# i2Nav-WHU/IC-GVINS

Measured on AMD Instinct MI355X. Metric: frames/s at 1280x720, 300 feats, 10-KF window; residual/Jacobian eval/s, higher is better.
Workload: dtype u8/int64 front-end (f32/f64 solves), f64 factors

## Files before the change

### ic-gvins_amd/csrc/ctx.hip

```cpp
#include <algorithm>
#include <cstdarg>

#include <sys/prctl.h>
#include <time.h>

#include "icg_internal.h"

int icg_fail(icg_ctx *ctx, int code, const char *fmt, ...) {
    char buf[512];
    va_list ap;
    va_start(ap, fmt);
    vsnprintf(buf, sizeof buf, fmt, ap);
    va_end(ap);
    if (ctx) ctx->err = buf;
    return code;
}

int icg_hip_check(icg_ctx *ctx, hipError_t e, const char *what) {
    if (e == hipSuccess) return 0;
    return icg_fail(ctx, ICG_ERR_HIP, "HIP error %d (%s) at %s", (int) e, hipGetErrorString(e), what);
}

static thread_local std::string g_create_error;

extern "C" const char *icg_version(void) { return "icgvins-hip 0.1 (gfx950)"; }

extern "C" const char *icg_last_error(const icg_ctx *ctx) { return ctx ? ctx->err.c_str() : g_create_error.c_str(); }

int icg_stream_wait_poll(icg_ctx *ctx) {
    static thread_local bool slack_set = false;
    if (!slack_set) {
        (void) prctl(PR_SET_TIMERSLACK, 1000UL, 0, 0, 0);
        slack_set = true;
    }
    struct timespec ts = {0, ctx->poll_sleep_ns};
    for (int it = 0;; it++) {
        hipError_t e = hipStreamQuery(ctx->stream);
        if (e == hipSuccess) return ICG_OK;
        if (e != hipErrorNotReady) return icg_hip_check(ctx, e, "hipStreamQuery");
        if (it >= 4) nanosleep(&ts, nullptr);
    }
}

extern "C" int icg_ctx_set_wait_mode(icg_ctx *ctx, int mode, int sleep_us) {
    if (!ctx || (mode != ICG_WAIT_SPIN && mode != ICG_WAIT_POLL) || (mode == ICG_WAIT_POLL && sleep_us <= 0)) return ICG_ERR_INVALID;
    if (ctx->wait_mode_env) return ICG_OK;
    ctx->poll_sleep_ns = mode == ICG_WAIT_POLL ? 1000L * sleep_us : 0;
    return ICG_OK;
}

icg_pyr_desc icg_make_pyr_desc(const icg_ctx *ctx) {
    icg_pyr_desc d{};
    d.base       = ctx->d_frames;
    d.slot_bytes = ctx->slot_bytes;
    d.n_levels   = ctx->n_levels;
    for (int l = 0; l < ICG_MAX_LEVELS; l++) {
        d.w[l]     = ctx->lv[l].w;
        d.h[l]     = ctx->lv[l].h;
        d.pitch[l] = ctx->lv[l].pitch;
        d.off[l]   = (unsigned int) ctx->lv[l].off;
    }
    return d;
}

extern "C" int icg_ctx_create(const icg_ctx_config *cfg, icg_ctx **out) {
    if (!cfg || !out) return ICG_ERR_INVALID;
    *out = nullptr;
    if (cfg->width < 32 || cfg->height < 32 || cfg->n_slots < 1 || cfg->max_batch < 1 || cfg->max_points < 1) {
        g_create_error = "icg_ctx_create: invalid configuration";
        return ICG_ERR_INVALID;
    }
    int ndev = 0;
    if (hipGetDeviceCount(&ndev) != hipSuccess || ndev <= 0 || cfg->device >= ndev) {
        g_create_error = "icg_ctx_create: no HIP device available (this library has no CPU fallback)";
        return ICG_ERR_NODEVICE;
    }
    icg_ctx *ctx = new icg_ctx();
    ctx->cfg     = *cfg;
    int rc       = 0;
    auto bail    = [&](int code) {
        g_create_error = ctx->err;
        icg_ctx_destroy(ctx);
        return code;
    };
    if ((rc = icg_hip_check(ctx, hipSetDevice(cfg->device), "hipSetDevice"))) return bail(rc);
    if ((rc = icg_hip_check(ctx, hipStreamCreateWithFlags(&ctx->stream, hipStreamNonBlocking), "hipStreamCreate")))
        return bail(rc);

    {
        const char *wm = getenv("ICG_WAIT_MODE");
        if (wm && strncmp(wm, "poll", 4) == 0) ctx->poll_sleep_ns = (wm[4] == ':' ? atol(wm + 5) : 20) * 1000L;
        ctx->wait_mode_env = wm != nullptr;
        if (wm && strcmp(wm, "block") == 0 &&
            (rc = icg_hip_check(ctx, hipEventCreateWithFlags(&ctx->ev_wait, hipEventBlockingSync | hipEventDisableTiming), "hipEventCreate")))
            return bail(rc);
    }

    int w = cfg->width, h = cfg->height;
    size_t off    = 0;
    ctx->n_levels = 0;
    for (int l = 0; l < ICG_MAX_LEVELS; l++) {
        if (l > 0) {
            w = (w + 1) / 2;
            h = (h + 1) / 2;
            if (w <= ICG_LK_WIN || h <= ICG_LK_WIN) break;
        }
        ctx->lv[l].w     = w;
        ctx->lv[l].h     = h;
        ctx->lv[l].pitch = (int) icg_align_up((size_t) w, 128);
        ctx->lv[l].off   = off;
        off += icg_align_up((size_t) ctx->lv[l].pitch * h, 256);
        ctx->n_levels++;
    }
    ctx->slot_bytes = off;
    for (int l = 0; l + 1 < ctx->n_levels; l++)
        if (ctx->lv[l].pitch % 4 != 0 || ctx->lv[l].off % 4 != 0 || ctx->lv[l].off + (size_t) ctx->lv[l].pitch * ctx->lv[l].h + 8 > ctx->slot_bytes ||
            ctx->lv[l].w < 8 || ctx->lv[l].h < 6 || ctx->lv[l].pitch < 16) {
            ctx->err = "icg_ctx_create: pyramid layout does not meet the row-stream kernel's invariants";
            return bail(ICG_ERR_INVALID);
        }
    ctx->raw_pitch  = ctx->lv[0].pitch;
    size_t tiles2   = (size_t) ICG_CLAHE_TILES * ICG_CLAHE_TILES;
// ... 225 lines not shown
```

### ic-gvins_amd/csrc/image.hip

```cpp
#include <algorithm>

#include "icg_internal.h"

#define PRE_MAX_JOBS 64
struct pre_jobs {
    const uint8_t *src[PRE_MAX_JOBS];
    int32_t slot[PRE_MAX_JOBS];
    int stride;
    const int32_t *slot_ind;
};
__device__ __forceinline__ int pre_job_slot(const pre_jobs &j, int b) { return j.slot_ind ? j.slot_ind[b] : j.slot[b]; }

__global__ void k_bgr2gray(const uint8_t *bgr, int w, int h, int sstride, size_t sbatch, uint8_t *gray, int gstride,
                           size_t gbatch) {
    int x = blockIdx.x * blockDim.x + threadIdx.x;
    int y = blockIdx.y;
    int b = blockIdx.z;
    if (x >= w) return;
    const uint8_t *p = bgr + (size_t) b * sbatch + (size_t) y * sstride + 3 * x;
    gray[(size_t) b * gbatch + (size_t) y * gstride + x] =
        (uint8_t) ((p[0] * 1868 + p[1] * 9617 + p[2] * 4899 + 8192) >> 14);
}

__global__ void k_hist256(pre_jobs jobs, int w, int h, unsigned int *hist ) {
// ... 124 lines not shown
            const unsigned int v = load_row_dword(r, x);
#pragma unroll
            for (int j = 0; j < 4; j++) {
                const int xx = x + j;
                if (xx >= x_begin && xx < x_end) atomicAdd(&hist[(v >> (8 * j)) & 0xff], 1u);
            }
        }
    }
    __syncthreads();

    const uint4 h4 = reinterpret_cast<const uint4 *>(hist)[lane];
    int hv[4]      = {(int) h4.x, (int) h4.y, (int) h4.z, (int) h4.w};
    int excess     = 0;
#pragma unroll
    for (int j = 0; j < 4; j++) {
        if (hv[j] > g.clip) {
            excess += hv[j] - g.clip;
            hv[j] = g.clip;
        }
    }
    const int clipped   = wave_sum_i32(excess);
    const int batch_add = clipped / 256;
    const int residual  = clipped - batch_add * 256;
    int step            = residual ? 256 / residual : 1;
    if (step < 1) step = 1;
    int run = 0;
#pragma unroll
    for (int j = 0; j < 4; j++) {
        const int t = 4 * lane + j;
        hv[j] += batch_add;
        if (residual != 0 && (t % step) == 0 && (t / step) < residual) hv[j]++;
        run += hv[j];
        hv[j] = run;
    }
    const int incl = wave_scan_i32(run);
    const int excl = incl - run;
    unsigned int packed = 0;
#pragma unroll
    for (int j = 0; j < 4; j++) {
        const float f = rintf((float) (excl + hv[j]) * g.lut_scale);
        int iv        = (int) f;
        iv            = iv < 0 ? 0 : (iv > 255 ? 255 : iv);
        packed |= (unsigned int) iv << (8 * j);
    }
    reinterpret_cast<unsigned int *>(lut + ((size_t) b * ICG_CLAHE_TILES * ICG_CLAHE_TILES + tile) * 256)[lane] = packed;
}

#define CLAHE_CHUNK 256
#define CLAHE_MAXCOLS 24
#define CLAHE_FCOLS 8

typedef float f32x2 __attribute__((ext_vector_type(2)));

template <bool FLT>
__device__ __forceinline__ void clahe_apply_body(const pre_jobs &jobs, const clahe_geom &g, const uint8_t *lut, uint8_t *frames, size_t slot_bytes,
                                                 int dpitch, unsigned int *slut, int strip, int chunk, int b, int t, int dslot, int p_lo, int npairs,
                                                 int x_begin) {
    const int T = ICG_CLAHE_TILES;
    int ty1 = strip - 1, ty2 = strip;
    if (ty1 < 0) ty1 = 0;
    if (ty2 > T - 1) ty2 = T - 1;
    const unsigned int *blut = reinterpret_cast<const unsigned int *>(lut + (size_t) b * T * T * 256);
    for (int i = t; i < npairs * 64; i += 256) {
        const int p = p_lo + (i >> 6), v4 = i & 63;
        int c1 = p - 1, c2 = p;
        if (c1 < 0) c1 = 0;
        if (c2 > T - 1) c2 = T - 1;
        const unsigned int A = blut[(ty1 * T + c1) * 64 + v4], B = blut[(ty1 * T + c2) * 64 + v4];
        const unsigned int C = blut[(ty2 * T + c1) * 64 + v4], D = blut[(ty2 * T + c2) * 64 + v4];
        if (FLT) {
            float4 *dst = reinterpret_cast<float4 *>(slut) + 4 * i;
#define CL_F(w, k) ((float) (((w) >> (8 * (k))) & 0xffu))
            dst[0] = make_float4(CL_F(A, 0), CL_F(B, 0), CL_F(C, 0), CL_F(D, 0));
            dst[1] = make_float4(CL_F(A, 1), CL_F(B, 1), CL_F(C, 1), CL_F(D, 1));
            dst[2] = make_float4(CL_F(A, 2), CL_F(B, 2), CL_F(C, 2), CL_F(D, 2));
            dst[3] = make_float4(CL_F(A, 3), CL_F(B, 3), CL_F(C, 3), CL_F(D, 3));
#undef CL_F
        } else {
            const unsigned int ab01 = __builtin_amdgcn_perm(B, A, 0x05010400u), ab23 = __builtin_amdgcn_perm(B, A, 0x07030602u);
            const unsigned int cd01 = __builtin_amdgcn_perm(D, C, 0x05010400u), cd23 = __builtin_amdgcn_perm(D, C, 0x07030602u);
            uint4 e;
            e.x = __builtin_amdgcn_perm(cd01, ab01, 0x05040100u);
            e.y = __builtin_amdgcn_perm(cd01, ab01, 0x07060302u);
            e.z = __builtin_amdgcn_perm(cd23, ab23, 0x05040100u);
            e.w = __builtin_amdgcn_perm(cd23, ab23, 0x07060302u);
            reinterpret_cast<uint4 *>(slut)[i] = e;
        }
    }
    __syncthreads();

    const int wave = t >> 6, lane = t & 63;
    const int x0 = x_begin + lane * 4;
    int pofs[4];
    float xa[4], xa1[4];
#pragma unroll
    for (int k = 0; k < 4; k++) {
        const int x     = x0 + k;
        const float txf = x * g.inv_tw - 0.5f;
        const int tx1   = (int) floorf(txf);
        xa[k]           = txf - tx1;
        xa1[k]          = 1.0f - xa[k];
        int p           = tx1 + 1 - p_lo;
        p               = p < 0 ? 0 : (p > npairs - 1 ? npairs - 1 : p);
        pofs[k]         = p << 8;
    }
    if (x0 >= g.w) return;

    int y_lo = (strip - 1) * g.th + g.th / 2 - 2;
    int y_hi = strip * g.th + g.th / 2 + 3;
    if (y_lo < 0) y_lo = 0;
    if (y_hi > g.h) y_hi = g.h;
    const uint8_t *src = jobs.src[b];
    const int stride   = jobs.stride;
    uint8_t *dst       = frames + (size_t) dslot * slot_bytes;
    if (FLT) {
        const float4 *sf = reinterpret_cast<const float4 *>(slut);
        for (int y = y_lo + wave; y < y_hi; y += 4) {
            const float tyf = y * g.inv_th - 0.5f;
            const int tyr   = (int) floorf(tyf);
            if (tyr != strip - 1) continue;
            const float ya = tyf - tyr, ya1 = 1.0f - ya;
            const unsigned int pin = *reinterpret_cast<const unsigned int *>(src + (size_t) y * stride + x0);
            const float4 e0 = sf[pofs[0] + (pin & 0xff)], e1 = sf[pofs[1] + ((pin >> 8) & 0xff)];
            const float4 e2 = sf[pofs[2] + ((pin >> 16) & 0xff)], e3 = sf[pofs[3] + (pin >> 24)];
            const float r0 = (e0.x * xa1[0] + e0.y * xa[0]) * ya1 + (e0.z * xa1[0] + e0.w * xa[0]) * ya;
            const float r1 = (e1.x * xa1[1] + e1.y * xa[1]) * ya1 + (e1.z * xa1[1] + e1.w * xa[1]) * ya;
            const float r2 = (e2.x * xa1[2] + e2.y * xa[2]) * ya1 + (e2.z * xa1[2] + e2.w * xa[2]) * ya;
            const float r3 = (e3.x * xa1[3] + e3.y * xa[3]) * ya1 + (e3.z * xa1[3] + e3.w * xa[3]) * ya;
            const unsigned int m0 = __float_as_uint(r0 + 12582912.f), m1 = __float_as_uint(r1 + 12582912.f);
            const unsigned int m2 = __float_as_uint(r2 + 12582912.f), m3 = __float_as_uint(r3 + 12582912.f);
            const unsigned int lo = __builtin_amdgcn_perm(m1, m0, 0x0c0c0400u), hi = __builtin_amdgcn_perm(m3, m2, 0x0c0c0400u);
            *reinterpret_cast<unsigned int *>(dst + (size_t) y * dpitch + x0) = __builtin_amdgcn_perm(hi, lo, 0x05040100u);
        }
        return;
    }
    const f32x2 XA01 = {xa[0], xa[1]}, XA23 = {xa[2], xa[3]}, XB01 = {xa1[0], xa1[1]}, XB23 = {xa1[2], xa1[3]};
    for (int y = y_lo + wave; y < y_hi; y += 4) {
        const float tyf = y * g.inv_th - 0.5f;
        const int tyr   = (int) floorf(tyf);
        if (tyr != strip - 1) continue;
        const float ya = tyf - tyr, ya1 = 1.0f - ya;
        const unsigned int pin = *reinterpret_cast<const unsigned int *>(src + (size_t) y * stride + x0);
        const unsigned int e0 = slut[pofs[0] + (pin & 0xff)], e1 = slut[pofs[1] + ((pin >> 8) & 0xff)];
        const unsigned int e2 = slut[pofs[2] + ((pin >> 16) & 0xff)], e3 = slut[pofs[3] + (pin >> 24)];
#define CL_B(e, k) ((float) (((e) >> (8 * (k))) & 0xffu))
        const f32x2 A01 = {CL_B(e0, 0), CL_B(e1, 0)}, B01 = {CL_B(e0, 1), CL_B(e1, 1)};
        const f32x2 C01 = {CL_B(e0, 2), CL_B(e1, 2)}, D01 = {CL_B(e0, 3), CL_B(e1, 3)};
        const f32x2 A23 = {CL_B(e2, 0), CL_B(e3, 0)}, B23 = {CL_B(e2, 1), CL_B(e3, 1)};
        const f32x2 C23 = {CL_B(e2, 2), CL_B(e3, 2)}, D23 = {CL_B(e2, 3), CL_B(e3, 3)};
#undef CL_B
        const f32x2 r01 = (A01 * XB01 + B01 * XA01) * ya1 + (C01 * XB01 + D01 * XA01) * ya;
        const f32x2 r23 = (A23 * XB23 + B23 * XA23) * ya1 + (C23 * XB23 + D23 * XA23) * ya;
        const float res[4] = {r01.x, r01.y, r23.x, r23.y};
        unsigned int pout = 0;
#pragma unroll
        for (int k = 0; k < 4; k++) {
            const int iv = (int) rintf(res[k]);
            pout |= (unsigned int) (iv < 0 ? 0 : (iv > 255 ? 255 : iv)) << (8 * k);
        }
        *reinterpret_cast<unsigned int *>(dst + (size_t) y * dpitch + x0) = pout;
    }
}

__global__ __launch_bounds__(256) void k_clahe_apply(pre_jobs jobs, clahe_geom g, const uint8_t *lut, uint8_t *frames,
                                                     size_t slot_bytes, int dpitch) {
    __shared__ __attribute__((aligned(16))) unsigned int slut[CLAHE_FCOLS * 256 * 4];
    static_assert(CLAHE_FCOLS * 4 >= CLAHE_MAXCOLS, "the byte form must fit the same array");
    const int strip = blockIdx.x;
    const int chunk = blockIdx.y;
    const int b     = blockIdx.z;
    const int t     = threadIdx.x;
    const int dslot = pre_job_slot(jobs, b);
    if (!jobs.src[b] || dslot < 0) return;
    const int x_begin = chunk * CLAHE_CHUNK;
    int x_end         = x_begin + CLAHE_CHUNK;
    if (x_end > g.w) x_end = g.w;
    const int p_lo   = (int) floorf(x_begin * g.inv_tw - 0.5f) + 1;
    const int p_hi   = (int) floorf((x_end - 1) * g.inv_tw - 0.5f) + 1;
    const int npairs = p_hi - p_lo + 1;
    if (npairs <= CLAHE_FCOLS)
        clahe_apply_body<true>(jobs, g, lut, frames, slot_bytes, dpitch, slut, strip, chunk, b, t, dslot, p_lo, npairs, x_begin);
    else
        clahe_apply_body<false>(jobs, g, lut, frames, slot_bytes, dpitch, slut, strip, chunk, b, t, dslot, p_lo, npairs, x_begin);
}

#define PR_STRIP_OUT 128
struct pr_sel {
    unsigned int a, b, t, v;
};
typedef unsigned int pr_u3 __attribute__((ext_vector_type(3)));
__device__ __forceinline__ pr_u3 pr_load(const uint8_t *row, unsigned int wx) {
    typedef pr_u3 __attribute__((aligned(4))) u3a;
    return *reinterpret_cast<const u3a *>(row + wx);
}
template <bool EDGE> __device__ __forceinline__ unsigned int pr_hsum(const pr_u3 E, const pr_sel &S) {
    unsigned int A, B, V4;
    if (EDGE) {
        A  = __builtin_amdgcn_perm(E.y, E.x, S.a);
        B  = __builtin_amdgcn_perm(E.y, E.x, S.b);
        V4 = __builtin_amdgcn_perm(E.z, __builtin_amdgcn_perm(E.y, E.x, S.t), S.v);
    } else {
        A  = __builtin_amdgcn_alignbyte(E.y, E.x, 2);
        B  = E.y;
        V4 = E.z & 0xffu;
    }
    const unsigned int h0 = __builtin_amdgcn_udot4(B, 0x00010000u, __builtin_amdgcn_udot4(A, 0x04060401u, 0u, false), false);
    const unsigned int h1 = __builtin_amdgcn_udot4(B, 0x04060401u, V4, false);
    return h0 | (h1 << 16);
}

template <bool EDGE>
__device__ __forceinline__ void pr_band(const uint8_t *src, int sh, int spitch, uint8_t *dst, int dpitch, int i0, int i1, unsigned int wx,
                                        const pr_sel &S, unsigned int dcol, bool store) {
    auto srow = [&](int r) { return src + (unsigned int) __builtin_amdgcn_readfirstlane(icg_reflect1(r, sh) * spitch); };
    unsigned int hA = pr_hsum<EDGE>(pr_load(srow(2 * i0 - 2), wx), S), hB = pr_hsum<EDGE>(pr_load(srow(2 * i0 - 1), wx), S);
    unsigned int hC = pr_hsum<EDGE>(pr_load(srow(2 * i0), wx), S);
    pr_u3 R1 = pr_load(srow(2 * i0 + 1), wx), R2 = pr_load(srow(2 * i0 + 2), wx);
    for (int i = i0; i < i1; i++) {
        const pr_u3 N1 = pr_load(srow(2 * i + 3), wx), N2 = pr_load(srow(2 * i + 4), wx);
        const unsigned int hD = pr_hsum<EDGE>(R1, S), hE = pr_hsum<EDGE>(R2, S);
        unsigned int v = hA + hE;
        v              = ((hB + hD) << 2) + v;
        v += (hC << 2) + (hC + hC);
        v += 0x00800080u;
        if (store) *reinterpret_cast<unsigned short *>(dst + (size_t) i * dpitch + dcol) = (unsigned short) __builtin_amdgcn_perm(v, v, 0x0c0c0301u);
        hA = hC, hB = hD, hC = hE;
        R1 = N1, R2 = N2;
    }
}

__global__ __launch_bounds__(64) void k_pyrdown_rows(uint8_t *frames, size_t slot_bytes, pre_jobs jobs, unsigned int src_off, int sw, int sh,
                                                     int spitch, unsigned int dst_off, int dw, int dh, int dpitch, int n_strips, int n_bands,
                                                     int band_rows, int n_tasks) {
    const int task = icg_xcd_chunked(blockIdx.x, n_tasks);
    if (task >= n_tasks) return;
    const int per_job = n_strips * n_bands;
// ... 198 lines not shown
```

### ic-gvins_amd/csrc/lk.hip

```cpp
#include <cfloat>

#include "dev_camera.h"
#include "icg_internal.h"

using namespace icgd;

#define LK_IT 24
#define LK_IS 28
#define LK_JT 32
#define LK_JS 36
#define LK_JM 5
#define LK_BW 28
#define LK_BH 26
#define LK_MAX_ITERS 30
#ifndef LK_WAVES_PER_EU
#define LK_WAVES_PER_EU 5
#endif

struct lk_smem {
    unsigned int I[LK_IT * LK_IS / 4];
    unsigned int J[LK_JT * LK_JS / 4 + 1];
    int B[LK_BH * LK_BW] __attribute__((aligned(16)));
};

// ... 65 lines not shown
}

__device__ __forceinline__ void wave_sum3_i32x16_f32(int v1, int v2, int v3, float &f1, float &f2, float &f3) {
    const int x       = lk_fold32(v1, v2);
    const int y       = lk_fold32(v3, 0);
    const lk_u2 r     = __builtin_amdgcn_permlane16_swap((unsigned int) x, (unsigned int) y, false, false);
    int v             = (int) (r.x + r.y);
    v                 = dpp_add_xor1(v);
    v                 = dpp_add_xor2(v);
    int hi = v >> 16, lo = v & 0xffff;
    hi                = dpp_add_half_mirror(hi);
    lo                = dpp_add_half_mirror(lo);
    hi                = dpp_add_mirror(hi);
    lo                = dpp_add_mirror(lo);
    const float t     = lk_combine_f32(hi, lo);
    f1                = lk_readlane_f32(t, 0);
    f3                = lk_readlane_f32(t, 16);
    f2                = lk_readlane_f32(t, 32);
}

__device__ __forceinline__ int lk_descale(int v, int n) { return (v + (1 << (n - 1))) >> n; }

__device__ __forceinline__ void lk_weights_pk(float a, float b, unsigned int &W0, unsigned int &W1) {
    const float A = a * (float) (1 << 14), A1 = (float) (1 << 14) - A, b1 = 1.f - b;
    const unsigned int r00 = __float_as_uint(A1 * b1 + 12582912.f), r01 = __float_as_uint(A * b1 + 12582912.f);
    const unsigned int r10 = __float_as_uint(A1 * b + 12582912.f);
    const unsigned int r11 = 0x4000u - (r00 + r01 + r10);
    W0 = __builtin_amdgcn_perm(r01, r00, 0x05040100u);
    W1 = __builtin_amdgcn_perm(r11, r10, 0x05040100u);
}

__device__ __forceinline__ void lk_weights(float a, float b, int &w00, int &w01, int &w10, int &w11) {
    const float A = a * (float) (1 << 14), A1 = (float) (1 << 14) - A, b1 = 1.f - b;
    w00 = (int) rintf(A1 * b1);
    w01 = (int) rintf(A * b1);
    w10 = (int) rintf(A1 * b);
    w11 = (1 << 14) - w00 - w01 - w10;
}

__device__ __forceinline__ unsigned int lk_load4(const unsigned char *row, int x, int W) {
    if (x >= 0 && x + 3 < W) {
        typedef unsigned int __attribute__((aligned(1))) u32u;
        return *reinterpret_cast<const u32u *>(row + x);
    }
    unsigned int v = 0;
#pragma unroll
    for (int k = 0; k < 4; k++) v |= (unsigned int) row[icg_reflect101(x + k, W)] << (8 * k);
    return v;
}
__device__ __forceinline__ int lk_byte(unsigned int w, int k) { return (int) ((w >> (8 * k)) & 0xffu); }

typedef unsigned int __attribute__((aligned(1))) lk_u32u;

__device__ __forceinline__ void lk_load_I(unsigned int (&v)[3], const unsigned char *I, int W, int H, int pitch, int ipx, int ipy,
                                          int lane) {
    const bool inside = ipx - 1 >= 0 && ipx - 1 + LK_IT <= W && ipy - 1 >= 0 && ipy - 1 + LK_IT <= H;
#pragma unroll
    for (int q = 0; q < 3; q++) {
        const int i = lane + 64 * q;
        const int r = i / 6, cd = i - r * 6;
        v[q] = 0;
        if (i < LK_IT * 6) {
            if (inside)
                v[q] = *reinterpret_cast<const lk_u32u *>(I + (size_t) (ipy - 1 + r) * pitch + (ipx - 1 + 4 * cd));
            else
                v[q] = lk_load4(I + (size_t) icg_reflect101(ipy - 1 + r, H) * pitch, ipx - 1 + 4 * cd, W);
        }
    }
}
__device__ __forceinline__ void lk_store_I(lk_smem &S, const unsigned int (&v)[3], int lane) {
#pragma unroll
    for (int q = 0; q < 3; q++) {
        const int i = lane + 64 * q;
        const int r = i / 6, cd = i - r * 6;
        if (i < LK_IT * 6) S.I[(r * LK_IS >> 2) + cd] = v[q];
    }
}
__device__ __forceinline__ void lk_load_J(unsigned int (&v)[4], const unsigned char *J, int W, int H, int pitch, int jx0, int jy0,
                                          int lane) {
    const int r = lane >> 1, c0 = (lane & 1) * 16;
    const bool inside = jx0 >= 0 && jx0 + LK_JT <= W && jy0 >= 0 && jy0 + LK_JT <= H;
    if (inside) {
        const unsigned char *row = J + (size_t) (jy0 + r) * pitch + (jx0 + c0);
#pragma unroll
        for (int q = 0; q < 4; q++) v[q] = *reinterpret_cast<const lk_u32u *>(row + 4 * q);
    } else {
        const unsigned char *row = J + (size_t) icg_reflect101(jy0 + r, H) * pitch;
#pragma unroll
        for (int q = 0; q < 4; q++) v[q] = lk_load4(row, jx0 + c0 + 4 * q, W);
    }
}
__device__ __forceinline__ void lk_store_J(lk_smem &S, const unsigned int (&v)[4], int lane) {
    const int r = lane >> 1, c0 = (lane & 1) * 16;
    unsigned int *dst = &S.J[(r * LK_JS + c0) >> 2];
#pragma unroll
    for (int q = 0; q < 4; q++) dst[q] = v[q];
}
__device__ __forceinline__ void lk_stage_J(lk_smem &S, const unsigned char *J, int W, int H, int pitch, int jx0, int jy0,
                                           int lane) {
    unsigned int v[4];
    lk_load_J(v, J, W, H, pitch, jx0, jy0, lane);
    lk_store_J(S, v, lane);
}

typedef short s16x2 __attribute__((ext_vector_type(2)));
typedef unsigned short u16x2 __attribute__((ext_vector_type(2)));

__device__ __forceinline__ unsigned int pk_add(unsigned int a, unsigned int b) {
    return __builtin_bit_cast(unsigned int, (u16x2) (__builtin_bit_cast(u16x2, a) + __builtin_bit_cast(u16x2, b)));
}
__device__ __forceinline__ unsigned int pk_sub(unsigned int a, unsigned int b) {
    return __builtin_bit_cast(unsigned int, (u16x2) (__builtin_bit_cast(u16x2, a) - __builtin_bit_cast(u16x2, b)));
}
__device__ __forceinline__ unsigned int pk_mul(unsigned int a, unsigned short k) {
    return __builtin_bit_cast(unsigned int, (u16x2) (__builtin_bit_cast(u16x2, a) * k));
}
__device__ __forceinline__ int dot2(unsigned int a, unsigned int b, int c) {
    return __builtin_amdgcn_sdot2(__builtin_bit_cast(s16x2, a), __builtin_bit_cast(s16x2, b), c, false);
}
__device__ __forceinline__ int dot2_keep(unsigned int a, unsigned int b, int c) {
    int d;
    asm("v_dot2_i32_i16 %0, %1, %2, %3" : "=v"(d) : "v"(a), "v"(b), "v"(c));
    return d;
}
__device__ __forceinline__ int dot2_keep_s(unsigned int a, unsigned int b, int c_uniform) {
    int d;
    asm("v_dot2_i32_i16 %0, %1, %2, %3" : "=v"(d) : "v"(a), "v"(b), "s"(c_uniform));
    return d;
}
__device__ __forceinline__ int dot2_zero(unsigned int a, unsigned int b) {
    int d;
    asm("v_dot2_i32_i16 %0, %1, %2, 0" : "=v"(d) : "v"(a), "v"(b));
    return d;
}
__device__ __forceinline__ int mad24_12(int a, int c) {
    int d;
    asm("v_mad_i32_i24 %0, %1, 12, %2" : "=v"(d) : "v"(a), "v"(c));
    return d;
}
__device__ __forceinline__ int mad24_40_s(int a, int c_uniform) {
    int d;
    asm("v_mad_i32_i24 %0, %1, 40, %2" : "=v"(d) : "v"(a), "s"(c_uniform));
    return d;
}
__device__ __forceinline__ unsigned int pk_lo16(int a, int b) {
    return __builtin_amdgcn_perm((unsigned int) b, (unsigned int) a, 0x05040100u);
}
__device__ __forceinline__ unsigned int pk_hi16(int a, int b) {
    return __builtin_amdgcn_perm((unsigned int) b, (unsigned int) a, 0x07060302u);
}
__device__ __forceinline__ unsigned int pk_shift(unsigned int a, unsigned int b) { return __builtin_amdgcn_alignbit(b, a, 16); }

__device__ __forceinline__ void lk_fetch_J(const lk_smem &S, int row0, int o, unsigned int (&JA)[7], unsigned int (&JB)[7]) {
    const int idx = o >> 2, sh = o & 3;
    const unsigned int *r0 = &S.J[(row0 * LK_JS >> 2) + idx];
    const unsigned int *r1 = r0 + (LK_JS >> 2);
    const unsigned int d0 = r0[0], d1 = r0[1], d2 = r0[2];
    const unsigned int e0 = r1[0], e1 = r1[1], e2 = r1[2];
    const unsigned int a0 = __builtin_amdgcn_alignbyte(d1, d0, sh), a1 = __builtin_amdgcn_alignbyte(d2, d1, sh);
    const unsigned int b0 = __builtin_amdgcn_alignbyte(e1, e0, sh), b1 = __builtin_amdgcn_alignbyte(e2, e1, sh);
#pragma unroll
    for (int k = 0; k < 7; k++) {
        const unsigned int sel = 0x0c000c00u | (unsigned int) k | ((unsigned int) (k + 1) << 16);
        JA[k] = __builtin_amdgcn_perm(a1, a0, sel);
        JB[k] = __builtin_amdgcn_perm(b1, b0, sel);
    }
}

__device__ __forceinline__ void lk_zero_rows(lk_smem &S, int lane) {
    static_assert(3 * LK_BW <= 128, "two stores per lane cover the rows of zeros");
    S.B[(LK_BH - 3) * LK_BW + lane] = 0;
    if (lane < 3 * LK_BW - 64) S.B[(LK_BH - 3) * LK_BW + 64 + lane] = 0;
}

__device__ bool lk_track_wave(const icg_pyr_desc &P, const unsigned char *slotI, const unsigned char *slotJ,
                              float2 prevPt, float2 &nextIO, lk_smem &S, int lane, float *err_out) {
    const float FLT_SCALE = 1.f / (1 << 20);
    const double eps2     = 0.01 * 0.01;
    bool status           = true;
    float errv            = 0.f;
    float2 nextStore      = nextIO;
    const int maxLevel    = P.n_levels - 1;
    const bool active     = lane < 63;
    const int ly          = active ? lane / 3 : 0;
    const int lx0         = active ? (lane - ly * 3) * 7 : 0;
    const unsigned int am = active ? ~0u : 0u;
    int rnd15 = 1 << 15, rnd8 = 1 << 8;
    asm volatile("" : "+s"(rnd15), "+s"(rnd8));

    for (int level = maxLevel; level >= 0; --level) {
        const int W = P.w[level], H = P.h[level], pitch = P.pitch[level];
        const unsigned char *I = slotI + P.off[level];
        const unsigned char *J = slotJ + P.off[level];
        const float scale      = (float) (1. / (1 << level));
        float prevx = prevPt.x * scale, prevy = prevPt.y * scale;
        float nptx, npty;
        if (level == maxLevel) {
            nptx = nextStore.x * scale;
            npty = nextStore.y * scale;
        } else {
            nptx = nextStore.x * 2.f;
            npty = nextStore.y * 2.f;
        }
        nextStore = make_float2(nptx, npty);

        prevx -= (float) ICG_LK_HALF;
        prevy -= (float) ICG_LK_HALF;
        const int ipx = (int) floorf(prevx), ipy = (int) floorf(prevy);
        if (ipx < -ICG_LK_WIN || ipx >= W || ipy < -ICG_LK_WIN || ipy >= H) {
            if (level == 0) {
                status = false;
                errv   = 0.f;
            }
            continue;
        }
        unsigned int W0, W1;
        lk_weights_pk(prevx - ipx, prevy - ipy, W0, W1);

        int jx0 = -1000000, jy0 = -1000000;
        {
            const int inx0 = (int) floorf(nptx - (float) ICG_LK_HALF), iny0 = (int) floorf(npty - (float) ICG_LK_HALF);
            const bool jok = !(inx0 < -ICG_LK_WIN || inx0 >= W || iny0 < -ICG_LK_WIN || iny0 >= H);
            unsigned int vi[3] = {0, 0, 0}, vj[4] = {0, 0, 0, 0};
            lk_load_I(vi, I, W, H, pitch, ipx, ipy, lane);
            if (jok) {
                jx0 = inx0 - LK_JM;
                jy0 = iny0 - LK_JM;
                lk_load_J(vj, J, W, H, pitch, jx0, jy0, lane);
            }
            __syncthreads();
            lk_store_I(S, vi, lane);
            if (jok) lk_store_J(S, vj, lane);
            __syncthreads();
        }

        int c0[7];
        unsigned int IXP[4], IYP[4];
        int sA11 = 0, sA12 = 0, sA22 = 0;
        float A11, A12, A22;
        const bool all_in = ipx >= 0 && ipx + 22 <= W && ipy >= 0 && ipy + 22 <= H;
        if (all_in) {
            asm volatile("" ::: "memory");
            {
                const int br = min(lane >> 1, 22), bs = lane & 1;
                const unsigned int *p = &S.I[(br * LK_IS >> 2) + 3 * bs];
                unsigned int d[2][4];
#pragma unroll
// ... 196 lines not shown
            const float ex = nextStore.x - (float) ICG_LK_HALF, ey = nextStore.y - (float) ICG_LK_HALF;
            const int inx = (int) floorf(ex), iny = (int) floorf(ey);
            if (inx < -ICG_LK_WIN || inx >= W || iny < -ICG_LK_WIN || iny >= H) {
                status = false;
                continue;
            }
            if (err_out) {
                if (inx != cinx || iny != ciny) {
                    if (!(inx >= jx0 && inx <= jx0 + (LK_JT - 22) && iny >= jy0 && iny <= jy0 + (LK_JT - 22))) {
                        jx0 = inx - LK_JM;
                        jy0 = iny - LK_JM;
                        __syncthreads();
                        lk_stage_J(S, J, W, H, pitch, jx0, jy0, lane);
                        __syncthreads();
                    }
                    lk_fetch_J(S, iny - jy0 + ly, (inx - jx0) + lx0, JA, JB);
                }
                lk_weights_pk(ex - inx, ey - iny, W0, W1);
                int se = 0;
#pragma unroll
                for (int k = 0; k < 7; k++) {
                    const int diff = dot2(JB[k], W1, dot2_keep(JA[k], W0, c0[k])) >> 9;
                    se += diff < 0 ? -diff : diff;
                }
                se &= (int) am;
                errv = wave_sum_i32x16_f32(se) * 1.f / (float) (32 * ICG_LK_WIN * ICG_LK_WIN);
            }
        }
    }
    nextIO = nextStore;
    if (err_out && lane == 0) *err_out = errv;
    return status;
}

__global__ __launch_bounds__(64) void k_lk_track(icg_pyr_desc P, int n, const int32_t *prev_slot, const int32_t *next_slot,
                                                 const float2 *prev_pts, float2 *next_pts, unsigned char *status, float *err) {
    __shared__ lk_smem S;
    const int i = icg_xcd_chunked(blockIdx.x, n);
    if (i >= n) return;
    const int lane = threadIdx.x;
    lk_zero_rows(S, lane);
    const unsigned char *sI = P.base + (size_t) prev_slot[i] * P.slot_bytes;
    const unsigned char *sJ = P.base + (size_t) next_slot[i] * P.slot_bytes;
    float2 nx = next_pts[i];
    bool st   = lk_track_wave(P, sI, sJ, prev_pts[i], nx, S, lane, err ? err + i : nullptr);
    if (lane == 0) {
        next_pts[i] = nx;
        status[i]   = st ? 1 : 0;
    }
}

__global__ __launch_bounds__(64, LK_WAVES_PER_EU) void k_lk_track_fb(icg_pyr_desc P, int n, const int32_t *prev_slot,
                                                    const int32_t *next_slot, const float2 *prev_pts,
                                                    const float2 *guess_pts, float2 *out_pts, unsigned char *status,
                                                    float2 *out_bwd, int img_w, int img_h,
                                                    int seg_cap, const int32_t *seg_count) {
    __shared__ lk_smem S;
    const int i = icg_xcd_chunked(blockIdx.x, n);
    if (i >= n) return;
    if (seg_count) {
        const int s = i / seg_cap;
        if (i - s * seg_cap >= seg_count[s]) return;
    }
    const int lane = threadIdx.x;
    lk_zero_rows(S, lane);
    const unsigned char *sP = P.base + (size_t) prev_slot[i] * P.slot_bytes;
    const unsigned char *sN = P.base + (size_t) next_slot[i] * P.slot_bytes;
    const float2 p0 = prev_pts[i];
    float2 fwd      = guess_pts[i];
    float2 bwd      = p0;
    bool st_f = false, st_b = false;
    for (int dir = 0; dir < 2; dir++) {
        if (dir) {
            const bool border = fwd.x < 5.f || fwd.y < 5.f || fwd.x > (float) (img_w - 5) || fwd.y > (float) (img_h - 5);
            if (!st_f || border) break;
        }
        const unsigned char *a = dir ? sN : sP, *b = dir ? sP : sN;
        const float2 from      = dir ? fwd : p0;
        float2 io              = dir ? bwd : fwd;
        const bool st          = lk_track_wave(P, a, b, from, io, S, lane, nullptr);
        if (dir) {
            bwd  = io;
            st_b = st;
        } else {
            fwd  = io;
            st_f = st;
        }
    }
    if (lane == 0) {
        out_pts[i] = fwd;
        out_bwd[i] = bwd;
        status[i]  = (unsigned char) ((st_f && st_b) ? 1u : 0u);
    }
}

__global__ __launch_bounds__(256) void k_lk_finish(int n, const float2 *prev_pts, const float2 *out_pts, float2 *bwd_undist, unsigned char *status,
                                                   int want_undist, int has_cam, icg_camera cam, int img_w, int img_h, int seg_cap,
                                                   const int32_t *seg_count) {
    const int i = blockIdx.x * 256 + threadIdx.x;
    if (i >= n) return;
    if (seg_count) {
        const int s = i / seg_cap;
        if (i - s * seg_cap >= seg_count[s]) return;
    }
    const float2 p0 = prev_pts[i], fwd = out_pts[i], bwd = bwd_undist[i];
    const bool border = (double) fwd.x < 5.0 || (double) fwd.y < 5.0 || ((double) fwd.x > (img_w - 5.0)) || ((double) fwd.y > (img_h - 5.0));
    const double ddx = (double) (bwd.x - p0.x), ddy = (double) (bwd.y - p0.y);
    const double dist = sqrt(ddx * ddx + ddy * ddy);
    status[i] = (unsigned char) ((status[i] && !border && dist < 0.5) ? 1u : 0u);
    if (want_undist) bwd_undist[i] = has_cam ? cam_undistort(cam, fwd) : fwd;
}

__global__ __launch_bounds__(1024) void k_keep_indices(int n, const unsigned char *status, int32_t *keep_idx, int32_t *n_keep) {
    __shared__ int wave_tot[16];
    __shared__ int base;
    const int t = threadIdx.x, lane = t & 63, wv = t >> 6;
    if (t == 0) base = 0;
    __syncthreads();
    for (int start = 0; start < n; start += 1024) {
        const int i   = start + t;
        const bool k  = i < n && status[i];
        const unsigned long long m = __ballot(k);
        const int pre = __popcll(m & ((1ull << lane) - 1ull));
        if (lane == 0) wave_tot[wv] = __popcll(m);
        __syncthreads();
        int off = base;
        for (int w = 0; w < wv; w++) off += wave_tot[w];
        if (k) keep_idx[off + pre] = i;
        __syncthreads();
        if (t == 0) {
            int s = 0;
            for (int w = 0; w < 16; w++) s += wave_tot[w];
            base += s;
        }
        __syncthreads();
    }
    if (t == 0) *n_keep = base;
}

static int check_slots(icg_ctx *ctx, int n, const int32_t *a, const int32_t *b) {
    for (int i = 0; i < n; i++)
        if (a[i] < 0 || a[i] >= ctx->cfg.n_slots || b[i] < 0 || b[i] >= ctx->cfg.n_slots)
            return icg_fail(ctx, ICG_ERR_INVALID, "slot index out of range at point %d", i);
    return 0;
}

extern "C" int icg_lk_track(icg_ctx *ctx, int n, const int32_t *prev_slot, const int32_t *next_slot, const float *prev_pts,
                            float *next_pts, uint8_t *status, float *err) {
    if (!ctx || n < 0) return ICG_ERR_INVALID;
    if (n == 0) return ICG_OK;
    if (!prev_slot || !next_slot || !prev_pts || !next_pts || !status) return ICG_ERR_INVALID;
    if (n > ctx->cfg.max_points) return icg_fail(ctx, ICG_ERR_CAPACITY, "%d points > max_points %d", n, ctx->cfg.max_points);
    int rc = check_slots(ctx, n, prev_slot, next_slot);
    if (rc) return rc;
    ICG_HIP(ctx, hipSetDevice(ctx->cfg.device));
    icg_call c(ctx);
    if ((rc = c.reserve((size_t) n * 64))) return rc;
    const int32_t *d_ps = c.in_zc(prev_slot, (size_t) n);
    const int32_t *d_ns = c.in_zc(next_slot, (size_t) n);
    const float2 *d_pp  = (const float2 *) c.in_zc(prev_pts, 2 * (size_t) n);
    float2 *d_np        = (float2 *) c.out_zc(next_pts, 2 * (size_t) n);
    memcpy(d_np, next_pts, sizeof(float) * 2 * (size_t) n);
    unsigned char *d_st = c.out_zc(status, (size_t) n);
    float *d_err        = err ? c.out_zc(err, (size_t) n) : nullptr;
    ICG_LAUNCH_GUARD(c);
    {
        icg_prof_scope ps(ctx, "lk_track");
        hipLaunchKernelGGL(k_lk_track, dim3(icg_xcd_grid(n)), dim3(64), 0, ctx->stream, icg_make_pyr_desc(ctx), n, d_ps, d_ns, d_pp, d_np,
                           d_st, d_err);
    }
    ICG_HIP(ctx, hipGetLastError());
    return c.finish();
}

static void lk_fb_launch(icg_ctx *ctx, int n, int seg_cap, const int32_t *seg_count, bool want_undist, const int32_t *prev_slot, const int32_t *next_slot,
                         const float2 *prev, const float2 *guess, float2 *out, uint8_t *status, float2 *bwd_undist) {
    {
        icg_prof_scope ps(ctx, "lk_track_fb");
        hipLaunchKernelGGL(k_lk_track_fb, dim3(icg_xcd_grid(n)), dim3(64), 0, ctx->stream, icg_make_pyr_desc(ctx), n, prev_slot, next_slot, prev, guess, out,
                           status, bwd_undist, ctx->cfg.width, ctx->cfg.height, seg_cap, seg_count);
    }
    {
        icg_prof_scope ps(ctx, "lk_finish");
        hipLaunchKernelGGL(k_lk_finish, dim3((n + 255) / 256), dim3(256), 0, ctx->stream, n, prev, (const float2 *) out, bwd_undist, status,
                           want_undist ? 1 : 0, ctx->has_cam ? 1 : 0, ctx->cam, ctx->cfg.width, ctx->cfg.height, seg_cap, seg_count);
    }
}

extern "C" int icg_lk_track_fb(icg_ctx *ctx, int n, const int32_t *prev_slot, const int32_t *next_slot,
                               const float *prev_pts, const float *guess_pts, float *out_pts, uint8_t *status,
                               float *out_undist, int32_t *keep_idx, int32_t *n_keep) {
    if (!ctx || n < 0) return ICG_ERR_INVALID;
    if (n == 0) {
        if (n_keep) *n_keep = 0;
        return ICG_OK;
    }
    if (!prev_slot || !next_slot || !prev_pts || !guess_pts || !out_pts || !status) return ICG_ERR_INVALID;
    if ((keep_idx == nullptr) != (n_keep == nullptr)) return ICG_ERR_INVALID;
    if (out_undist && !ctx->has_cam) return icg_fail(ctx, ICG_ERR_INVALID, "out_undist requested but camera not set");
    if (n > ctx->cfg.max_points) return icg_fail(ctx, ICG_ERR_CAPACITY, "%d points > max_points %d", n, ctx->cfg.max_points);
    int rc = check_slots(ctx, n, prev_slot, next_slot);
    if (rc) return rc;
    ICG_HIP(ctx, hipSetDevice(ctx->cfg.device));
    icg_call c(ctx);
    if ((rc = c.reserve((size_t) n * 104))) return rc;
    const int32_t *d_ps = c.in_zc(prev_slot, (size_t) n);
    const int32_t *d_ns = c.in_zc(next_slot, (size_t) n);
    const float2 *d_pp  = (const float2 *) c.in_zc(prev_pts, 2 * (size_t) n);
    const float2 *d_gs  = (const float2 *) c.in_zc(guess_pts, 2 * (size_t) n);
    float2 *d_out       = (float2 *) c.out_zc(out_pts, 2 * (size_t) n);
    unsigned char *d_st = c.out_zc(status, (size_t) n);
    float2 *d_und       = out_undist ? (float2 *) c.out_zc(out_undist, 2 * (size_t) n) : (float2 *) c.out<float>(nullptr, 2 * (size_t) n);
    int32_t *d_keep     = keep_idx ? c.out_zc(keep_idx, (size_t) n) : nullptr;
    int32_t *d_nkeep    = keep_idx ? c.out_zc(n_keep, 1) : nullptr;
    ICG_LAUNCH_GUARD(c);
    lk_fb_launch(ctx, n, 0, nullptr, out_undist != nullptr, d_ps, d_ns, d_pp, d_gs, d_out, d_st, d_und);
    if (keep_idx) {
        icg_prof_scope ps(ctx, "keep_indices");
        hipLaunchKernelGGL(k_keep_indices, dim3(1), dim3(1024), 0, ctx->stream, n, d_st, d_keep, d_nkeep);
    }
    ICG_HIP(ctx, hipGetLastError());
    return c.finish();
}

int icg_lk_launch_segments(icg_ctx *ctx, int n_seg, int seg_cap, const int32_t *d_count, const int32_t *d_prev_slot, const int32_t *d_next_slot,
                           const float2 *d_prev, const float2 *d_guess, float2 *d_out, uint8_t *d_status, float2 *d_undist) {
    if (!ctx->has_cam) return icg_fail(ctx, ICG_ERR_INVALID, "camera not set");
    lk_fb_launch(ctx, n_seg * seg_cap, seg_cap, d_count, true, d_prev_slot, d_next_slot, d_prev, d_guess, d_out, d_status, d_undist);
    ICG_HIP(ctx, hipGetLastError());
    return ICG_OK;
}
```

### ic-gvins_amd/icgvins.py

```python
import ctypes as C
import os

import numpy as np

_HERE = os.path.dirname(os.path.abspath(__file__))
LIB_PATH = os.path.join(_HERE, "libicgvins_hip.so")

EXPORTS = [
    "icg_ctx_create", "icg_ctx_destroy", "icg_last_error", "icg_ctx_sync", "icg_ctx_set_wait_mode", "icg_ctx_stream", "icg_set_camera",
    "icg_version", "icg_pyramid_levels", "icg_prof_enable", "icg_prof_get", "icg_prof_names", "icg_dev_alloc",
    "icg_dev_free", "icg_dev_upload", "icg_dev_download", "icg_frames_preprocess", "icg_frame_download",
    "icg_lk_track", "icg_lk_track_fb", "icg_undistort_points", "icg_distort_points", "icg_predict_mappoints",
    "icg_predict_rotation", "icg_fm_ransac", "icg_fm_ransac_device", "icg_detect", "icg_triangulate", "icg_reproj_eval_batch",
    "icg_reproj_set_factors", "icg_reproj_stage_factors", "icg_reproj_commit_factors", "icg_reproj_eval_resident", "icg_reproj_accumulate_normal", "icg_preint_batch", "icg_preint_evaluate_batch",
    "icg_ins_mechanize_batch", "icg_ins_camera_pose_batch", "icg_reproj_schur", "icg_reproj_backsub", "icg_reproj_cost", "icg_reproj_landmark_diag",
    "icg_reproj_error_batch", "icg_reproj_set_windows", "icg_reproj_eval_windows", "icg_reproj_schur_windows",
    "icg_reproj_schur_windows_view", "icg_reproj_reserve_windows", "icg_reproj_eval_resident_view", "icg_reproj_backsub_windows", "icg_reproj_cost_windows", "icg_reproj_fetch_residuals", "icg_reproj_chi2_cull",
    "icg_reproj_landmark_diag_windows",
    "icg_marg_prior_set", "icg_marg_prior_evaluate", "icg_marg_linearize_batch",
    "icg_chol_solve_batch", "icg_reproj_schur_windows_resident", "icg_reproj_solve_windows", "icg_reproj_host_parts_build",
]


MARG_MAX_R = 1024
# ... 76 lines not shown
        except Exception:
            pass

    def _ck(self, rc, what):
        if rc != 0:
            raise IcgError(f"{what} failed rc={rc}: {self.lib.icg_last_error(self.h).decode()}")

    def sync(self):
        self._ck(self.lib.icg_ctx_sync(self.h), "icg_ctx_sync")

    def levels(self):
        return self.lib.icg_pyramid_levels(self.h)

    def set_camera(self, cam10):
        cam = Camera(*[float(v) for v in cam10])
        self._ck(self.lib.icg_set_camera(self.h, C.byref(cam)), "icg_set_camera")

    def prof_enable(self, on=True):
        self._ck(self.lib.icg_prof_enable(self.h, 1 if on else 0), "icg_prof_enable")

    def prof(self):
        buf = C.create_string_buffer(4096)
        self._ck(self.lib.icg_prof_names(self.h, buf, 4096), "icg_prof_names")
        out = {}
        for name in buf.value.decode().split("\n"):
            if not name:
                continue
            n, ms = C.c_int(), C.c_double()
            self.lib.icg_prof_get(self.h, name.encode(), C.byref(n), C.byref(ms))
            out[name] = (n.value, ms.value)
        return out

    def dev_alloc(self, nbytes):
        p = C.c_void_p()
        self._ck(self.lib.icg_dev_alloc(self.h, C.c_size_t(nbytes), C.byref(p)), "icg_dev_alloc")
        return p.value

    def dev_free(self, ptr):
        self._ck(self.lib.icg_dev_free(self.h, C.c_void_p(ptr)), "icg_dev_free")

    def dev_upload(self, ptr, arr):
        arr = np.ascontiguousarray(arr)
        self._ck(self.lib.icg_dev_upload(self.h, C.c_void_p(ptr), _p(arr), C.c_size_t(arr.nbytes)), "icg_dev_upload")

    def preprocess(self, slots, images, want_hist=False):
        n = len(slots)
        imgs = [np.ascontiguousarray(im, dtype=np.uint8) for im in images]
        ch = 3 if imgs[0].ndim == 3 else 1
        stride = imgs[0].strides[0]
        ptrs = (C.c_void_p * n)(*[im.ctypes.data for im in imgs])
        hist = np.zeros(n, np.float64) if want_hist else None
        self._ck(self.lib.icg_frames_preprocess(self.h, n, _p(_i32(slots)), ptrs, stride, ch, 0, _p(hist)),
                 "icg_frames_preprocess")
        return hist

    def preprocess_device(self, slots, dev_ptrs, stride, channels=1):
        n = len(slots)
        ptrs = (C.c_void_p * n)(*dev_ptrs)
        self._ck(self.lib.icg_frames_preprocess(self.h, n, _p(_i32(slots)), ptrs, stride, channels, 1, None),
                 "icg_frames_preprocess")

    def download(self, slot, level=0):
        w, h = self.width, self.height
        for _ in range(level):
            w, h = (w + 1) // 2, (h + 1) // 2
        out = np.zeros((h, w), np.uint8)
        self._ck(self.lib.icg_frame_download(self.h, slot, level, _p(out), w), "icg_frame_download")
        return out

    def lk_track(self, prev_slot, next_slot, prev_pts, guess, want_err=True):
        prev_pts = _f32(prev_pts).reshape(-1, 2)
        n = prev_pts.shape[0]
        nxt = _f32(guess).reshape(-1, 2).copy()
        st = np.zeros(n, np.uint8)
        err = np.zeros(n, np.float32) if want_err else None
        ps = _i32(np.broadcast_to(prev_slot, (n,)))
        ns = _i32(np.broadcast_to(next_slot, (n,)))
        self._ck(self.lib.icg_lk_track(self.h, n, _p(ps), _p(ns), _p(prev_pts), _p(nxt), _p(st), _p(err)), "icg_lk_track")
        return nxt, st, err

    def lk_track_fb(self, prev_slot, next_slot, prev_pts, guess, want_undist=False, want_keep=False):
        prev_pts = _f32(prev_pts).reshape(-1, 2)
        guess = _f32(guess).reshape(-1, 2)
        n = prev_pts.shape[0]
        out = np.zeros((n, 2), np.float32)
        st = np.zeros(n, np.uint8)
        und = np.zeros((n, 2), np.float32) if want_undist else None
        keep = np.zeros(max(n, 1), np.int32) if want_keep else None
        nkeep = np.zeros(1, np.int32) if want_keep else None
        ps = _i32(np.broadcast_to(prev_slot, (n,)))
        ns = _i32(np.broadcast_to(next_slot, (n,)))
        self._ck(self.lib.icg_lk_track_fb(self.h, n, _p(ps), _p(ns), _p(prev_pts), _p(guess), _p(out), _p(st), _p(und),
                                           _p(keep), _p(nkeep)), "icg_lk_track_fb")
        res = [out, st]
        if want_undist:
            res.append(und)
        if want_keep:
            res.append(keep[:int(nkeep[0])])
        return tuple(res)

    def undistort(self, pts):
        p = _f32(pts).reshape(-1, 2).copy()
        self._ck(self.lib.icg_undistort_points(self.h, p.shape[0], _p(p)), "icg_undistort_points")
        return p

    def distort(self, pts):
# ... 364 lines not shown
```

Measured before the change: 163,500.

## Tabulate CLAHE row weights and use 24-bit/magic-number index math in LK

The CLAHE apply kernel now precomputes per-row vertical interpolation weights into a small shared table, so the inner row loop no longer does floor/multiply per row, and the wave index is made scalar. The LK kernels switch address arithmetic to 24-bit multiplies, compute the level scale by exponent bit construction, and replace the segment division with a magic-number divide. Guards are added to reject image sizes and segment counts that would overflow the narrower arithmetic. The Python preprocess path now syncs when it passed temporary converted buffers, which fixes a lifetime hazard but adds a host wait.

```diff
diff --git a/ic-gvins_amd/csrc/ctx.hip b/ic-gvins_amd/csrc/ctx.hip
--- a/ic-gvins_amd/csrc/ctx.hip
+++ b/ic-gvins_amd/csrc/ctx.hip
@@ -68,6 +68,11 @@
     *out = nullptr;
     if (cfg->width < 32 || cfg->height < 32 || cfg->n_slots < 1 || cfg->max_batch < 1 || cfg->max_points < 1) {
         g_create_error = "icg_ctx_create: invalid configuration";
+        return ICG_ERR_INVALID;
+    }
+    if (cfg->width >= (1 << 24) || cfg->height >= (1 << 24) ||
+        (unsigned long long) icg_align_up((size_t) cfg->width, 128) * (unsigned long long) cfg->height >= (1ull << 31)) {
+        g_create_error = "icg_ctx_create: image too large: pitch * height of a pyramid level must stay below 2^31 bytes (32-bit tile offsets of the LK kernels)";
         return ICG_ERR_INVALID;
     }
     int ndev = 0;
diff --git a/ic-gvins_amd/csrc/image.hip b/ic-gvins_amd/csrc/image.hip
--- a/ic-gvins_amd/csrc/image.hip
+++ b/ic-gvins_amd/csrc/image.hip
@@ -200,7 +200,26 @@
 
 typedef float f32x2 __attribute__((ext_vector_type(2)));
 
-template <bool FLT>
+#define CLAHE_ROWS 128
+__device__ __forceinline__ float2 clahe_row_entry(const float2 *rows, int y, int y_lo, int y_hi) {
+    const int r = min(y, y_hi - 1) - y_lo;
+    return rows[r < 0 ? 0 : r];
+}
+template <bool TAB>
+__device__ __forceinline__ bool clahe_row(const float2 *rows, float2 &next, int y, int y_lo, int y_hi, float inv_th, int strip, float &ya, float &ya1) {
+    if (TAB) {
+        ya = next.x, ya1 = next.y;
+        next = clahe_row_entry(rows, y + 4, y_lo, y_hi);
+        return ya1 >= 0.f;
+    }
+    const float tyf = y * inv_th - 0.5f;
+    const int tyr   = (int) floorf(tyf);
+    ya              = tyf - tyr;
+    ya1             = 1.0f - ya;
+    return tyr == strip - 1;
+}
+
+template <bool FLT, bool TAB>
 __device__ __forceinline__ void clahe_apply_body(const pre_jobs &jobs, const clahe_geom &g, const uint8_t *lut, uint8_t *frames, size_t slot_bytes,
                                                  int dpitch, unsigned int *slut, int strip, int chunk, int b, int t, int dslot, int p_lo, int npairs,
                                                  int x_begin) {
@@ -208,6 +227,17 @@
     int ty1 = strip - 1, ty2 = strip;
     if (ty1 < 0) ty1 = 0;
     if (ty2 > T - 1) ty2 = T - 1;
+    int y_lo = (strip - 1) * g.th + g.th / 2 - 2;
+    int y_hi = strip * g.th + g.th / 2 + 3;
+    if (y_lo < 0) y_lo = 0;
+    if (y_hi > g.h) y_hi = g.h;
+    float2 *rows = reinterpret_cast<float2 *>(slut + CLAHE_FCOLS * 256 * 4) - CLAHE_ROWS;
+    if (TAB && t < y_hi - y_lo) {
+        float ya, ya1;
+        float2 none = make_float2(0.f, 0.f);
+        const bool mine = clahe_row<false>(nullptr, none, y_lo + t, y_lo, y_hi, g.inv_th, strip, ya, ya1);
+        rows[t] = make_float2(ya, mine ? ya1 : -1.f);
+    }
     const unsigned int *blut = reinterpret_cast<const unsigned int *>(lut + (size_t) b * T * T * 256);
     for (int i = t; i < npairs * 64; i += 256) {
         const int p = p_lo + (i >> 6), v4 = i & 63;
@@ -237,7 +267,7 @@
     }
     __syncthreads();
 
-    const int wave = t >> 6, lane = t & 63;
+    const int wave = __builtin_amdgcn_readfirstlane(t >> 6), lane = t & 63;
     const int x0 = x_begin + lane * 4;
     int pofs[4];
     float xa[4], xa1[4];
@@ -254,20 +284,15 @@
     }
     if (x0 >= g.w) return;
 
-    int y_lo = (strip - 1) * g.th + g.th / 2 - 2;
-    int y_hi = strip * g.th + g.th / 2 + 3;
-    if (y_lo < 0) y_lo = 0;
-    if (y_hi > g.h) y_hi = g.h;
     const uint8_t *src = jobs.src[b];
     const int stride   = jobs.stride;
     uint8_t *dst       = frames + (size_t) dslot * slot_bytes;
+    float2 next        = TAB ? clahe_row_entry(rows, y_lo + wave, y_lo, y_hi) : make_float2(0.f, 0.f);
     if (FLT) {
         const float4 *sf = reinterpret_cast<const float4 *>(slut);
         for (int y = y_lo + wave; y < y_hi; y += 4) {
-            const float tyf = y * g.inv_th - 0.5f;
-            const int tyr   = (int) floorf(tyf);
-            if (tyr != strip - 1) continue;
-            const float ya = tyf - tyr, ya1 = 1.0f - ya;
+            float ya, ya1;
+            if (!clahe_row<TAB>(rows, next, y, y_lo, y_hi, g.inv_th, strip, ya, ya1)) continue;
             const unsigned int pin = *reinterpret_cast<const unsigned int *>(src + (size_t) y * stride + x0);
             const float4 e0 = sf[pofs[0] + (pin & 0xff)], e1 = sf[pofs[1] + ((pin >> 8) & 0xff)];
             const float4 e2 = sf[pofs[2] + ((pin >> 16) & 0xff)], e3 = sf[pofs[3] + (pin >> 24)];
@@ -284,10 +309,8 @@
     }
     const f32x2 XA01 = {xa[0], xa[1]}, XA23 = {xa[2], xa[3]}, XB01 = {xa1[0], xa1[1]}, XB23 = {xa1[2], xa1[3]};
     for (int y = y_lo + wave; y < y_hi; y += 4) {
-        const float tyf = y * g.inv_th - 0.5f;
-        const int tyr   = (int) floorf(tyf);
-        if (tyr != strip - 1) continue;
-        const float ya = tyf - tyr, ya1 = 1.0f - ya;
+        float ya, ya1;
+        if (!clahe_row<TAB>(rows, next, y, y_lo, y_hi, g.inv_th, strip, ya, ya1)) continue;
         const unsigned int pin = *reinterpret_cast<const unsigned int *>(src + (size_t) y * stride + x0);
         const unsigned int e0 = slut[pofs[0] + (pin & 0xff)], e1 = slut[pofs[1] + ((pin >> 8) & 0xff)];
         const unsigned int e2 = slut[pofs[2] + ((pin >> 16) & 0xff)], e3 = slut[pofs[3] + (pin >> 24)];
@@ -326,10 +349,17 @@
     const int p_lo   = (int) floorf(x_begin * g.inv_tw - 0.5f) + 1;
     const int p_hi   = (int) floorf((x_end - 1) * g.inv_tw - 0.5f) + 1;
     const int npairs = p_hi - p_lo + 1;
-    if (npairs <= CLAHE_FCOLS)
-        clahe_apply_body<true>(jobs, g, lut, frames, slot_bytes, dpitch, slut, strip, chunk, b, t, dslot, p_lo, npairs, x_begin);
+    static_assert(CLAHE_ROWS * sizeof(float2) <= 256 * 4 * 4 && CLAHE_MAXCOLS * 256 * 4 + CLAHE_ROWS * sizeof(float2) <= sizeof(slut) && CLAHE_ROWS <= 256,
+                  "the row table must fit behind CLAHE_FCOLS - 1 float pairs and behind the byte form, one thread per row");
+    const bool tab = g.th + 5 <= CLAHE_ROWS;
+    if (npairs < CLAHE_FCOLS && tab)
+        clahe_apply_body<true, true>(jobs, g, lut, frames, slot_bytes, dpitch, slut, strip, chunk, b, t, dslot, p_lo, npairs, x_begin);
+    else if (npairs <= CLAHE_FCOLS)
+        clahe_apply_body<true, false>(jobs, g, lut, frames, slot_bytes, dpitch, slut, strip, chunk, b, t, dslot, p_lo, npairs, x_begin);
+    else if (tab)
+        clahe_apply_body<false, true>(jobs, g, lut, frames, slot_bytes, dpitch, slut, strip, chunk, b, t, dslot, p_lo, npairs, x_begin);
     else
-        clahe_apply_body<false>(jobs, g, lut, frames, slot_bytes, dpitch, slut, strip, chunk, b, t, dslot, p_lo, npairs, x_begin);
+        clahe_apply_body<false, false>(jobs, g, lut, frames, slot_bytes, dpitch, slut, strip, chunk, b, t, dslot, p_lo, npairs, x_begin);
 }
 
 #define PR_STRIP_OUT 128
diff --git a/ic-gvins_amd/csrc/lk.hip b/ic-gvins_amd/csrc/lk.hip
--- a/ic-gvins_amd/csrc/lk.hip
+++ b/ic-gvins_amd/csrc/lk.hip
@@ -141,6 +141,10 @@
 
 typedef unsigned int __attribute__((aligned(1))) lk_u32u;
 
+__device__ __forceinline__ unsigned int lk_offset(int row, int pitch, int col) {
+    return __umul24((unsigned int) row, (unsigned int) pitch) + (unsigned int) col;
+}
+
 __device__ __forceinline__ void lk_load_I(unsigned int (&v)[3], const unsigned char *I, int W, int H, int pitch, int ipx, int ipy,
                                           int lane) {
     const bool inside = ipx - 1 >= 0 && ipx - 1 + LK_IT <= W && ipy - 1 >= 0 && ipy - 1 + LK_IT <= H;
@@ -151,7 +155,7 @@
         v[q] = 0;
         if (i < LK_IT * 6) {
             if (inside)
-                v[q] = *reinterpret_cast<const lk_u32u *>(I + (size_t) (ipy - 1 + r) * pitch + (ipx - 1 + 4 * cd));
+                v[q] = *reinterpret_cast<const lk_u32u *>(I + lk_offset(ipy - 1 + r, pitch, ipx - 1 + 4 * cd));
             else
                 v[q] = lk_load4(I + (size_t) icg_reflect101(ipy - 1 + r, H) * pitch, ipx - 1 + 4 * cd, W);
         }
@@ -170,7 +174,7 @@
     const int r = lane >> 1, c0 = (lane & 1) * 16;
     const bool inside = jx0 >= 0 && jx0 + LK_JT <= W && jy0 >= 0 && jy0 + LK_JT <= H;
     if (inside) {
-        const unsigned char *row = J + (size_t) (jy0 + r) * pitch + (jx0 + c0);
+        const unsigned char *row = J + lk_offset(jy0 + r, pitch, jx0 + c0);
 #pragma unroll
         for (int q = 0; q < 4; q++) v[q] = *reinterpret_cast<const lk_u32u *>(row + 4 * q);
     } else {
@@ -242,7 +246,7 @@
 
 __device__ __forceinline__ void lk_fetch_J(const lk_smem &S, int row0, int o, unsigned int (&JA)[7], unsigned int (&JB)[7]) {
     const int idx = o >> 2, sh = o & 3;
-    const unsigned int *r0 = &S.J[(row0 * LK_JS >> 2) + idx];
+    const unsigned int *r0 = &S.J[__umul24((unsigned int) row0, LK_JS >> 2) + (unsigned int) idx];
     const unsigned int *r1 = r0 + (LK_JS >> 2);
     const unsigned int d0 = r0[0], d1 = r0[1], d2 = r0[2];
     const unsigned int e0 = r1[0], e1 = r1[1], e2 = r1[2];
@@ -281,7 +285,7 @@
         const int W = P.w[level], H = P.h[level], pitch = P.pitch[level];
         const unsigned char *I = slotI + P.off[level];
         const unsigned char *J = slotJ + P.off[level];
-        const float scale      = (float) (1. / (1 << level));
+        const float scale      = __uint_as_float((unsigned int) (127 - level) << 23);
         float prevx = prevPt.x * scale, prevy = prevPt.y * scale;
         float nptx, npty;
         if (level == maxLevel) {
@@ -584,14 +588,14 @@
 
 __global__ __launch_bounds__(64, LK_WAVES_PER_EU) void k_lk_track_fb(icg_pyr_desc P, int n, const int32_t *prev_slot,
                                                     const int32_t *next_slot, const float2 *prev_pts,
-                                                    const float2 *guess_pts, float2 *out_pts, unsigned char *status,
-                                                    float2 *out_bwd, int img_w, int img_h,
-                                                    int seg_cap, const int32_t *seg_count) {
+                                                    const float2 *guess_pts, int img_w, int img_h,
+                                                    int seg_cap, unsigned int seg_magic, const int32_t *seg_count,
+                                                    float2 *out_pts, unsigned char *status, float2 *out_bwd) {
     __shared__ lk_smem S;
     const int i = icg_xcd_chunked(blockIdx.x, n);
     if (i >= n) return;
     if (seg_count) {
-        const int s = i / seg_cap;
+        const int s = icg_div_by_magic(i, seg_magic);
         if (i - s * seg_cap >= seg_count[s]) return;
     }
     const int lane = threadIdx.x;
@@ -628,11 +632,11 @@
 
 __global__ __launch_bounds__(256) void k_lk_finish(int n, const float2 *prev_pts, const float2 *out_pts, float2 *bwd_undist, unsigned char *status,
                                                    int want_undist, int has_cam, icg_camera cam, int img_w, int img_h, int seg_cap,
-                                                   const int32_t *seg_count) {
+                                                   unsigned int seg_magic, const int32_t *seg_count) {
     const int i = blockIdx.x * 256 + threadIdx.x;
     if (i >= n) return;
     if (seg_count) {
-        const int s = i / seg_cap;
+        const int s = icg_div_by_magic(i, seg_magic);
         if (i - s * seg_cap >= seg_count[s]) return;
     }
     const float2 p0 = prev_pts[i], fwd = out_pts[i], bwd = bwd_undist[i];
@@ -707,15 +711,16 @@
 
 static void lk_fb_launch(icg_ctx *ctx, int n, int seg_cap, const int32_t *seg_count, bool want_undist, const int32_t *prev_slot, const int32_t *next_slot,
                          const float2 *prev, const float2 *guess, float2 *out, uint8_t *status, float2 *bwd_undist) {
+    const unsigned int seg_magic = seg_count ? icg_div_magic(seg_cap) : 0u;
     {
         icg_prof_scope ps(ctx, "lk_track_fb");
-        hipLaunchKernelGGL(k_lk_track_fb, dim3(icg_xcd_grid(n)), dim3(64), 0, ctx->stream, icg_make_pyr_desc(ctx), n, prev_slot, next_slot, prev, guess, out,
-                           status, bwd_undist, ctx->cfg.width, ctx->cfg.height, seg_cap, seg_count);
+        hipLaunchKernelGGL(k_lk_track_fb, dim3(icg_xcd_grid(n)), dim3(64), 0, ctx->stream, icg_make_pyr_desc(ctx), n, prev_slot, next_slot, prev, guess,
+                           ctx->cfg.width, ctx->cfg.height, seg_cap, seg_magic, seg_count, out, status, bwd_undist);
     }
     {
         icg_prof_scope ps(ctx, "lk_finish");
         hipLaunchKernelGGL(k_lk_finish, dim3((n + 255) / 256), dim3(256), 0, ctx->stream, n, prev, (const float2 *) out, bwd_undist, status,
-                           want_undist ? 1 : 0, ctx->has_cam ? 1 : 0, ctx->cam, ctx->cfg.width, ctx->cfg.height, seg_cap, seg_count);
+                           want_undist ? 1 : 0, ctx->has_cam ? 1 : 0, ctx->cam, ctx->cfg.width, ctx->cfg.height, seg_cap, seg_magic, seg_count);
     }
 }
 
@@ -758,6 +763,8 @@
 int icg_lk_launch_segments(icg_ctx *ctx, int n_seg, int seg_cap, const int32_t *d_count, const int32_t *d_prev_slot, const int32_t *d_next_slot,
                            const float2 *d_prev, const float2 *d_guess, float2 *d_out, uint8_t *d_status, float2 *d_undist) {
     if (!ctx->has_cam) return icg_fail(ctx, ICG_ERR_INVALID, "camera not set");
+    if (n_seg < 1 || seg_cap < 1 || (unsigned long long) n_seg * seg_cap * seg_cap >= (1ull << 32))
+        return icg_fail(ctx, ICG_ERR_INVALID, "%d segments of %d entries: the segment decode needs n_seg * seg_cap^2 < 2^32", n_seg, seg_cap);
     lk_fb_launch(ctx, n_seg * seg_cap, seg_cap, d_count, true, d_prev_slot, d_next_slot, d_prev, d_guess, d_out, d_status, d_undist);
     ICG_HIP(ctx, hipGetLastError());
     return ICG_OK;
diff --git a/ic-gvins_amd/icgvins.py b/ic-gvins_amd/icgvins.py
--- a/ic-gvins_amd/icgvins.py
+++ b/ic-gvins_amd/icgvins.py
@@ -152,6 +152,8 @@
         hist = np.zeros(n, np.float64) if want_hist else None
         self._ck(self.lib.icg_frames_preprocess(self.h, n, _p(_i32(slots)), ptrs, stride, ch, 0, _p(hist)),
                  "icg_frames_preprocess")
+        if hist is None and any(a is not b for a, b in zip(imgs, images)):
+            self.sync()
         return hist
 
     def preprocess_device(self, slots, dev_ptrs, stride, channels=1):
```

Measured after the change: 166,000 (median of 6 runs). 1.02x the previous value.
